# halajun/diasss

Hardware: NVIDIA B200
Metric: image-pairs/sec (extract+match) (higher is better)
Workload: dtype u8

## Files before the change

diasss_b200/csrc/fast.cu:

```cuda
#include <cuda.h>
#include <cuda_fp16.h>
#include <cuda_pipeline.h>

#include <algorithm>
#include <cstring>
#include <vector>

#include "dsx_internal.cuh"

namespace dsx {

namespace {

#ifndef DSX_FAST_WARPS
#define DSX_FAST_WARPS 8
#endif
constexpr int kWarps = DSX_FAST_WARPS;
constexpr int kLX = 8 * kWarps;
constexpr int kLXs = (kWarps == 8) ? 6 : (kWarps == 4) ? 5 : 4;
static_assert((1 << kLXs) == kLX, "kWarps must be 2, 4 or 8");
constexpr int kPad = 4;

#ifndef DSX_FAST_FP16
#define DSX_FAST_FP16 1
#endif
#ifndef DSX_FAST_END_FMA
#define DSX_FAST_END_FMA 8
#endif

__device__ __forceinline__ uint32_t ld4(const uint8_t* s, int off) {
    const uint32_t* w = reinterpret_cast<const uint32_t*>(s + (off & ~3));
    return __funnelshift_r(w[0], w[1], (off & 3) * 8);
}

template <int S>
__device__ __forceinline__ uint32_t win(uint32_t P, uint32_t Q, uint32_t N) {
    if (S == 0) return P;
    if (S < 4) return __funnelshift_r(P, Q, 8 * S);
    if (S == 4) return Q;
    if (S < 8) return __funnelshift_r(Q, N, 8 * (S - 4));
    return N;
}

#if !DSX_FAST_FP16
__device__ __forceinline__ uint32_t arc_pair(const uint32_t (&r)[16], uint32_t c, uint32_t t_floor) {
    uint32_t pn[8], px[8];
#pragma unroll
    for (int j = 0; j < 8; j++) {
        pn[j] = __vminu2(r[2 * j + 1], r[(2 * j + 2) & 15]);
        px[j] = __vmaxu2(r[2 * j + 1], r[(2 * j + 2) & 15]);
    }
    uint32_t qn[8], qx[8];
#pragma unroll
    for (int j = 0; j < 8; j++) {
        qn[j] = __vminu2(pn[j], pn[(j + 1) & 7]);
        qx[j] = __vmaxu2(px[j], px[(j + 1) & 7]);
    }
    uint32_t wn[8], wx[8];
#pragma unroll
    for (int j = 0; j < 8; j++) {
        const uint32_t en = __vmaxu2(r[2 * j], r[(2 * j + 9) & 15]), ex = __vminu2(r[2 * j], r[(2 * j + 9) & 15]);
        wn[j] = __vimin3_u16x2(qn[j], qn[(j + 2) & 7], en);
        wx[j] = __vimax3_u16x2(qx[j], qx[(j + 2) & 7], ex);
    }
    uint32_t a = __vimax3_u16x2(__vimax3_u16x2(wn[0], wn[1], wn[2]), __vimax3_u16x2(wn[3], wn[4], wn[5]), __vmaxu2(wn[6], wn[7]));
    uint32_t b = __vimin3_u16x2(__vimin3_u16x2(wx[0], wx[1], wx[2]), __vimin3_u16x2(wx[3], wx[4], wx[5]), __vminu2(wx[6], wx[7]));
    const uint32_t A = __byte_perm(a, 0, 0x4341), B = __byte_perm(b, 0, 0x4341), C = __byte_perm(c, 0, 0x4341);
    const uint32_t X = A + 0x80008000u - C, Y = C + 0x80008000u - B;
    return __vimax3_u16x2(X, Y, 0x80008000u + t_floor * 0x00010001u) - 0x80018001u;
}

#endif

__device__ __forceinline__ void hminmax(uint32_t a, uint32_t b, uint32_t& mn, uint32_t& mx) {
    const __half2 ha = *reinterpret_cast<const __half2*>(&a), hb = *reinterpret_cast<const __half2*>(&b);
    const __half2 d = __hfma2_relu(hb, __float2half2_rn(-1.0f), ha);
    const __half2 hx = __hadd2(hb, d), hn = __hsub2(ha, d);
    mx = *reinterpret_cast<const uint32_t*>(&hx);
    mn = *reinterpret_cast<const uint32_t*>(&hn);
}

__device__ __forceinline__ uint32_t arc_pair_h(const uint32_t (&r)[16], uint32_t c, uint32_t floor_bits) {
    uint32_t pn[8], px[8];
#pragma unroll
    for (int j = 0; j < 8; j++) hminmax(r[2 * j + 1], r[(2 * j + 2) & 15], pn[j], px[j]);
    uint32_t qn[8], qx[8];
#pragma unroll
    for (int j = 0; j < 8; j++) {
        qn[j] = __vminu2(pn[j], pn[(j + 1) & 7]);
        qx[j] = __vmaxu2(px[j], px[(j + 1) & 7]);
    }
    uint32_t wn[8], wx[8];
#pragma unroll
    for (int j = 0; j < 8; j++) {
        uint32_t en, ex;
        if (j < DSX_FAST_END_FMA) hminmax(r[2 * j], r[(2 * j + 9) & 15], ex, en);
        else { en = __vmaxu2(r[2 * j], r[(2 * j + 9) & 15]); ex = __vminu2(r[2 * j], r[(2 * j + 9) & 15]); }
        wn[j] = __vimin3_u16x2(qn[j], qn[(j + 2) & 7], en);
        wx[j] = __vimax3_u16x2(qx[j], qx[(j + 2) & 7], ex);
    }
    const uint32_t a = __vimax3_u16x2(__vimax3_u16x2(wn[0], wn[1], wn[2]), __vimax3_u16x2(wn[3], wn[4], wn[5]), __vmaxu2(wn[6], wn[7]));
    const uint32_t b = __vimin3_u16x2(__vimin3_u16x2(wx[0], wx[1], wx[2]), __vimin3_u16x2(wx[3], wx[4], wx[5]), __vminu2(wx[6], wx[7]));
    const __half2 ha = *reinterpret_cast<const __half2*>(&a), hb = *reinterpret_cast<const __half2*>(&b);
    const __half2 hc = *reinterpret_cast<const __half2*>(&c);
    const __half2 k256 = __float2half2_rn(256.0f);
    const __half2 X = __hadd2(ha, __hsub2(k256, hc)), Y = __hsub2(__hadd2(hc, k256), hb);
    const uint32_t m = __vimax3_u16x2(*reinterpret_cast<const uint32_t*>(&X), *reinterpret_cast<const uint32_t*>(&Y), floor_bits);
    const __half2 sc = __hadd2(*reinterpret_cast<const __half2*>(&m), __float2half2_rn(767.0f));
    return *reinterpret_cast<const uint32_t*>(&sc);
}

__device__ __forceinline__ void zero_score_border(uint8_t* score, int SP, int hd, int tid) {
    const int W = SP >> 2;
    uint32_t* sc = reinterpret_cast<uint32_t*>(score);
    for (int i = tid; i < 2 * W; i += kWarps * 32) sc[i < W ? i : (hd + 1) * W + (i - W)] = 0;
}

#ifdef DSX_FAST_PROFILE
__device__ unsigned long long g_fast_prof[512][16];
#define FAST_MARK(ph) do { if ((threadIdx.x & 31) == 0) { const long long t_ = clock64(); unsigned long long* s_ = g_fast_prof[(blockIdx.x * 8 + (threadIdx.x >> 5) + blockIdx.y * 37) & 511]; atomicAdd(s_ + 2 * (ph), (unsigned long long)(t_ - t_prev)); atomicAdd(s_ + 2 * (ph) + 1, 1ull); t_prev = t_; } } while (0)
#else
#define FAST_MARK(ph) do { } while (0)
#endif

struct FastArgs {
    LevelGeom g;
    const uint8_t* img;
    long long img_stride;
    int pitch;
    int32_t* cell_count;
    uint32_t* stage;
    long long cells_total, stage_total;
    int ini_th, min_th;
    int SP;
    int strip_bytes, score_bytes, list_bytes;
    int32_t* hist;
    unsigned long long* gbest;
    long long hist_total;
    const uint16_t* xlut;
    const uint8_t* ylut;
    int use_tma;
    CUtensorMap tmap;
};

constexpr int kFastMaxLevels = 8;
struct FastArgsAll {
    FastArgs lv[kFastMaxLevels];
    int first[kFastMaxLevels + 1];
    int nlevels;
};

__device__ __forceinline__ uint32_t smem_u32(const void* p) { return (uint32_t)__cvta_generic_to_shared(p); }

template <int SPC>
__global__ void __launch_bounds__(kWarps * 32, 32 / kWarps) fast_cells_kernel(const __grid_constant__ FastArgsAll AA) {
    int level = 0;
    while (level + 1 < AA.nlevels && (int)blockIdx.x >= AA.first[level + 1]) level++;
    const FastArgs& A = AA.lv[level];
    const int bx = (int)blockIdx.x - AA.first[level];
    extern __shared__ __align__(128) uint8_t smem[];
    __shared__ __align__(8) unsigned long long tma_bar;
#ifdef DSX_FAST_PROFILE
    long long t_prev = clock64();
#endif
    const LevelGeom& g = A.g;
    const int groupsX = (g.nCols + kWarps - 1) / kWarps;
    const int ci = bx / groupsX;
    const int j0 = (bx % groupsX) * kWarps;
    const int iniY = kMinBorder + ci * g.hCell;
    if (iniY >= g.maxBY - 3) return;
    const int maxY = min(iniY + g.hCell + 6, g.maxBY);
    const int hROI = maxY - iniY, hd = hROI - 6;
    int ncell = min(kWarps, g.nCols - j0);
    while (ncell > 0 && kMinBorder + (j0 + ncell - 1) * g.wCell >= g.maxBX - 6) ncell--;
    if (ncell == 0 || hd <= 0) return;
    const int xBegin = kMinBorder + j0 * g.wCell;
    const int xEnd = min(kMinBorder + (j0 + ncell) * g.wCell + 6, g.maxBX);
    const int xa = xBegin & ~3;
    const int xorg = A.use_tma ? ((xa - kPad) & ~15) : (xa - kPad);
    const int SP = SPC ? SPC : A.SP;
    uint8_t* strip = smem;
#if DSX_FAST_FP16
    uint8_t* score = smem;
    uint32_t* planeE = reinterpret_cast<uint32_t*>(smem + A.strip_bytes);
    uint32_t* planeO = planeE + (A.strip_bytes >> 1);
#else
    uint8_t* score = smem + 4 * A.strip_bytes;
#endif
    const uint8_t* img = A.img + (long long)blockIdx.y * A.img_stride;
    const int tid = threadIdx.x;

    if (A.use_tma == 2) {
        const uint32_t bar = smem_u32(&tma_bar);
        if (tid == 0) {
            asm volatile("mbarrier.init.shared::cta.b64 [%0], 1;" ::"r"(bar));
            asm volatile("fence.mbarrier_init.release.cluster;" ::: "memory");
            asm volatile("mbarrier.arrive.expect_tx.shared::cta.b64 _, [%0], %1;" ::"r"(bar), "r"((uint32_t)(SP * (g.hCell + 6))) : "memory");
            asm volatile("cp.async.bulk.tensor.3d.shared::cluster.global.mbarrier::complete_tx::bytes [%0], [%1, {%2, %3, %4}], [%5];"
                         ::"r"(smem_u32(strip)), "l"(&A.tmap), "r"(xorg >> 2), "r"(iniY), "r"((int)blockIdx.y), "r"(bar) : "memory");
        }
#if !DSX_FAST_FP16
        zero_score_border(score, SP, hd, tid);
#endif
        __syncthreads();
        if (tid < 32) {
            uint32_t done = 0;
            while (!done)
                asm volatile("{\n .reg .pred p;\n mbarrier.try_wait.parity.shared::cta.b64 p, [%1], %2;\n selp.u32 %0, 1, 0, p;\n}"
                             : "=r"(done) : "r"(bar), "r"(0u) : "memory");
        }
    } else if (A.use_tma) {
        const uint32_t bar = smem_u32(&tma_bar);
        const uint32_t row_bytes = (uint32_t)min(SP, A.pitch - xorg);
        if (tid == 0) {
            asm volatile("mbarrier.init.shared::cta.b64 [%0], 1;" ::"r"(bar));
            asm volatile("fence.mbarrier_init.release.cluster;" ::: "memory");
            asm volatile("mbarrier.arrive.expect_tx.shared::cta.b64 _, [%0], %1;" ::"r"(bar), "r"(row_bytes * (uint32_t)hROI) : "memory");
        }
        __syncthreads();
        if (tid < 32)
            for (int r = tid; r < hROI; r += 32)
                asm volatile("cp.async.bulk.shared::cluster.global.mbarrier::complete_tx::bytes [%0], [%1], %2, [%3];"
                             ::"r"(smem_u32(strip + r * SP)), "l"(img + (long long)(iniY + r) * A.pitch + xorg), "r"(row_bytes), "r"(bar) : "memory");
#if !DSX_FAST_FP16
        zero_score_border(score, SP, hd, tid);
#endif
        if (tid < 32) {
            uint32_t done = 0;
            while (!done)
                asm volatile("{\n .reg .pred p;\n mbarrier.try_wait.parity.shared::cta.b64 p, [%1], %2;\n selp.u32 %0, 1, 0, p;\n}"
                             : "=r"(done) : "r"(bar), "r"(0u) : "memory");
        }
    } else {
        const int nwords = (xEnd - xa + 3) >> 2;
        const int total = nwords * hROI;
        const int step_r = (kWarps * 32) / nwords, step_w = (kWarps * 32) - step_r * nwords;
        int r = tid / nwords, w = tid - r * nwords;
        for (int e = tid; e < total; e += kWarps * 32) {
            __pipeline_memcpy_async(strip + r * SP + (xa - xorg) + 4 * w, img + (long long)(iniY + r) * A.pitch + xa + 4 * w, 4);
            r += step_r; w += step_w;
            if (w >= nwords) { w -= nwords; r++; }
        }
        __pipeline_commit();
#if !DSX_FAST_FP16
        zero_score_border(score, SP, hd, tid);
#endif
        __pipeline_wait_prior(0);
    }
    FAST_MARK(0);
    __syncthreads();
    FAST_MARK(1);

#if DSX_FAST_FP16
    {
        const uint32_t* s0 = reinterpret_cast<const uint32_t*>(strip);
        const int total = (SP >> 2) * hROI;
        const uint32_t K = 0x64646464u;
        for (int e = tid; e < total; e += kWarps * 32) {
            const uint32_t a = s0[e], b = s0[e + 1];
            uint2 E, O;
            E.x = __byte_perm(a, K, 0x4140); E.y = __byte_perm(a, K, 0x4342);
            O.x = __byte_perm(a, K, 0x4241); O.y = __byte_perm(__byte_perm(a, b, 0x0043), K, 0x4140);
            *reinterpret_cast<uint2*>(planeE + 2 * e) = E;
            *reinterpret_cast<uint2*>(planeO + 2 * e) = O;
        }
    }
    FAST_MARK(2);
    __syncthreads();
    FAST_MARK(3);
    zero_score_border(score, SP, hd, tid);

    const uint32_t t_lo = (uint32_t)max(min(A.ini_th, A.min_th), 1);
    {
        constexpr int kPX = kWarps * 16;
        const int d0 = xBegin + 3 - xorg, d1 = xEnd - 3 - xorg;
        const int p0 = d0 >> 1, npx = ((d1 + 1) >> 1) - p0;
        const int W2 = SP >> 1;
        const __half2 fl = __float2half2_rn((float)(t_lo + 256));
        const uint32_t floor_bits = *reinterpret_cast<const uint32_t*>(&fl);
        for (int px = tid & (kPX - 1); px < npx; px += kPX) {
            const int e = p0 + px;
            uint32_t keep = 0xffffu;
            if (2 * e < d0) keep &= 0xff00u;
            if (2 * e + 1 >= d1) keep &= 0x00ffu;
            const int half = (hd + 1) >> 1;
            const int rbeg = (tid / kPX) ? half : 0, rend = (tid / kPX) ? hd : half;
            const uint32_t* qe = planeE + (rbeg + 3) * W2 + e;
            const uint32_t* qo = planeO + (rbeg + 3) * W2 + e;
            uint16_t* o = reinterpret_cast<uint16_t*>(score + (rbeg + 1) * SP) + e;
            uint32_t Rm = qo[-W2 + 1], Rc = qo[1], Lm = qo[-W2 - 2], Lc = qo[-2];
#pragma unroll 3
            for (int row = rbeg; row < rend; row++, qe += W2, qo += W2, o += SP >> 1) {
                uint32_t r[16];
                const uint32_t Rp = qo[W2 + 1], Lp = qo[W2 - 2];
#define RING(k, dx, dy) r[k] = ((dx) & 1) ? qo[(dy) * W2 + (((dx) - 1) >> 1)] : qe[(dy) * W2 + ((dx) >> 1)];
                RING(0, 0, 3)   RING(1, 1, 3)   RING(2, 2, 2)    r[3] = Rp;
                r[4] = Rc;      r[5] = Rm;      RING(6, 2, -2)   RING(7, 1, -3)
                RING(8, 0, -3)  RING(9, -1, -3) RING(10, -2, -2) r[11] = Lm;
                r[12] = Lc;     r[13] = Lp;     RING(14, -2, 2)  RING(15, -1, 3)
#undef RING
                const uint32_t sc = arc_pair_h(r, qe[0], floor_bits);
                *o = (uint16_t)(__byte_perm(sc, 0, 0x4420) & keep);
                Rm = Rc; Rc = Rp; Lm = Lc; Lc = Lp;
            }
        }
    }
#else
    {
        const uint32_t* s0 = reinterpret_cast<const uint32_t*>(strip);
        const int cw = A.strip_bytes >> 2;
        uint32_t* s1 = reinterpret_cast<uint32_t*>(strip) + cw;
        const int total = (SP >> 2) * hROI;
        for (int e = tid; e < total; e += kWarps * 32) {
            const uint32_t a = s0[e], b = s0[e + 1];
            s1[e] = __funnelshift_r(a, b, 8);
            s1[e + cw] = __funnelshift_r(a, b, 16);
            s1[e + 2 * cw] = __funnelshift_r(a, b, 24);
        }
    }
    FAST_MARK(2);
    __syncthreads();
    FAST_MARK(3);

    const uint32_t t_lo = (uint32_t)max(min(A.ini_th, A.min_th), 1);
    {
        const int d0 = xBegin + 3 - xorg, d1 = xEnd - 3 - xorg;
        const int w0 = d0 >> 2, nwx = ((d1 + 3) >> 2) - w0;
        const int W = SP >> 2, CW = A.strip_bytes >> 2;
        for (int wx = tid & (kLX - 1); wx < nwx; wx += kLX) {
            const int col = (w0 + wx) << 2;
            uint32_t keep = 0xffffffffu;
            if (d0 - col > 0) keep &= 0xffffffffu << (8 * (d0 - col));
            if (d1 - col < 4) keep &= 0xffffffffu >> (8 * (4 - (d1 - col)));
            const uint32_t* q = reinterpret_cast<const uint32_t*>(strip + ((tid >> kLXs) + 3) * SP + col);
            uint32_t* o = reinterpret_cast<uint32_t*>(score + ((tid >> kLXs) + 1) * SP + col);
            for (int row = tid >> kLXs; row < hd; row += (kWarps * 32) >> kLXs, q += 4 * W, o += 4 * W) {
                uint32_t ro[16], re[16];
#define WIN(S, dy) q[((S) & 3) * CW + (dy) * W + ((S) >> 2) - 1]
#define RING(k, dx, dy) { ro[k] = WIN(4 + (dx), dy); re[k] = WIN(3 + (dx), dy); }
                RING(0, 0, 3)   RING(1, 1, 3)   RING(2, 2, 2)    RING(3, 3, 1)
                RING(4, 3, 0)   RING(5, 3, -1)  RING(6, 2, -2)   RING(7, 1, -3)
                RING(8, 0, -3)  RING(9, -1, -3) RING(10, -2, -2) RING(11, -3, -1)
                RING(12, -3, 0) RING(13, -3, 1) RING(14, -2, 2)  RING(15, -1, 3)
#undef RING
                const uint32_t co = WIN(4, 0), ce = WIN(3, 0);
#undef WIN
                const uint32_t se = arc_pair(re, ce, t_lo);
                const uint32_t so = arc_pair(ro, co, t_lo);
                *o = (so * 256u + se) & keep;
            }
        }
    }
#endif
    FAST_MARK(4);
    __syncthreads();
    FAST_MARK(5);

    const int warp = tid >> 5, lane = tid & 31;
    if (warp >= ncell) return;
    const int cj = j0 + warp;
    const int iniX = kMinBorder + cj * g.wCell;
    const int maxX = min(iniX + g.wCell + 6, g.maxBX);
    const int wd = (maxX - iniX) - 6;
    const long long cell = g.cell_base + (long long)ci * g.nCols + cj;
    int32_t* out_count = A.cell_count + (long long)blockIdx.y * A.cells_total + cell;
    uint32_t* out_stage = A.stage + (long long)blockIdx.y * A.stage_total + g.stage_base +
                          ((long long)ci * g.nCols + cj) * g.cell_cap;
    if (wd <= 0) return;
    uint16_t* clist = reinterpret_cast<uint16_t*>(smem + A.strip_bytes + warp * A.list_bytes);
    const int sc0 = SP + (iniX + 3 - xorg);

    int ncorner = 0;
    const int nw = (wd + 3) >> 2;
    const uint32_t tail_mask = (wd & 3) ? ((1u << (8 * (wd & 3))) - 1u) : 0xffffffffu;
    for (int rbase = 0; rbase < hd; rbase += 32) {
        const int row = rbase + lane;
        uint32_t m_lo = 0, m_hi = 0;
        if (row < hd) {
            const int rb = sc0 + row * SP;
            uint32_t prev = 0, v = ld4(score, rb);
            if (nw == 1) v &= tail_mask;
            for (int wx = 0; wx < nw; wx++) {
                uint32_t next = 0;
                if (wx + 1 < nw) { next = ld4(score, rb + 4 * wx + 4); if (wx + 2 == nw) next &= tail_mask; }
                const uint32_t yl = __funnelshift_r(prev, v, 24), yr = __funnelshift_r(v, next, 8);
                const uint32_t xl = v & 0x7f7f7f7fu;
                const uint32_t tl = (yl | 0x80808080u) - xl, tr = (yr | 0x80808080u) - xl;
                const uint32_t gel = (yl & ~v) | (~(yl ^ v) & tl), ger = (yr & ~v) | (~(yr ^ v) & tr);
                const uint32_t gt = ~(gel | ger) & 0x80808080u;
                const uint32_t nib = (((gt >> 7) * 0x00204081u) >> 21) & 0xfu;
                if (wx < 8) m_lo |= nib << (4 * wx); else m_hi |= nib << (4 * wx - 32);
                prev = v; v = next;
            }
        }
        const int cnt = __popc(m_lo) + __popc(m_hi);
        int incl = cnt;
#pragma unroll
        for (int o = 1; o < 32; o <<= 1) { const int t = __shfl_up_sync(0xffffffffu, incl, o); if (lane >= o) incl += t; }
        int pos = ncorner + incl - cnt;
        while (m_lo) { clist[pos++] = (uint16_t)((row << 6) | (__ffs(m_lo) - 1)); m_lo &= m_lo - 1; }
        while (m_hi) { clist[pos++] = (uint16_t)((row << 6) | (__ffs(m_hi) + 31)); m_hi &= m_hi - 1; }
        ncorner += __shfl_sync(0xffffffffu, incl, 31);
    }
    __syncwarp();

    int cnt = 0;
    for (int pass = 0; pass < 2 && cnt == 0; pass++) {
        const int th = pass ? A.min_th : A.ini_th;
        for (int base = 0; base < ncorner; base += 32) {
            const int i = base + lane;
            bool emit = false; int idx = 0, s = 0;
            if (i < ncorner) {
                idx = clist[i];
                const int lx = idx & 63;
                const uint8_t* q = score + sc0 + (idx >> 6) * SP + lx;
                s = q[0];
                if (s >= th) {
                    const bool hasl = lx > 0, hasr = lx < wd - 1;
                    const int l0 = hasl ? q[-SP - 1] : 0, l2 = hasl ? q[SP - 1] : 0;
                    const int r0 = hasr ? q[-SP + 1] : 0, r2 = hasr ? q[SP + 1] : 0;
                    emit = s > l0 && s > l2 && s > r0 && s > r2 && s > q[-SP] && s > q[SP];
                }
            }
            const unsigned b = __ballot_sync(0xffffffffu, emit);
            if (emit) {
                const int e = cnt + __popc(b & ((1u << lane) - 1));
                out_stage[e] = (uint32_t)((idx & 63) + 3) | ((uint32_t)((idx >> 6) + 3) << 8) | ((uint32_t)s << 16);
                clist[e] = (uint16_t)idx;
            }
            cnt += __popc(b);
        }
        __syncwarp();
    }
    {
        int32_t* hist = A.hist + (long long)blockIdx.y * A.hist_total + g.hist_base;
        unsigned long long* gbest = A.gbest + (long long)blockIdx.y * A.hist_total + g.hist_base;
        const int ox = cj * g.wCell + 3, oy = ci * g.hCell + 3;
        const unsigned long long cl = (unsigned long long)(ci * g.nCols + cj);
        for (int base = 0; base < cnt; base += 32) {
            const int e = base + lane;
            unsigned code = 0xffffffffu, v = 0;
            if (e < cnt) {
                const int idx = clist[e];
                const unsigned xl = __ldg(A.xlut + ox + (idx & 63));
                code = ((xl >> 8) << (2 * g.qt_depth)) + ((unsigned)__ldg(A.ylut + oy + (idx >> 6)) << g.qt_depth) + (xl & 0xff);
                v = ((unsigned)score[sc0 + (idx >> 6) * SP + (idx & 63)] << 12) | (unsigned)(0xfff - e);
            }
            const unsigned peers = __match_any_sync(0xffffffffu, code);
            const unsigned mv = __reduce_max_sync(peers, v);
            if (e < cnt && lane == __ffs(peers) - 1) {
                atomicAdd(hist + code, __popc(peers));
                atomicMax(gbest + code, ((unsigned long long)(mv >> 12) << 56) | (kBestOrderMask - ((cl << 12) | (0xfff - (mv & 0xfff)))));
            }
        }
    }
    if (lane == 0) *out_count = cnt;
    FAST_MARK(6);
}

}

int fast_profile_read(unsigned long long* out16, int reset) {
#ifdef DSX_FAST_PROFILE
    std::vector<unsigned long long> h(512 * 16);
    if (cudaMemcpyFromSymbol(h.data(), g_fast_prof, sizeof(unsigned long long) * h.size()) != cudaSuccess) return DSX_ERR_CUDA;
    for (int k = 0; k < 16; k++) { out16[k] = 0; for (int s = 0; s < 512; s++) out16[k] += h[s * 16 + k]; }
    if (reset) {
        std::fill(h.begin(), h.end(), 0ull);
        if (cudaMemcpyToSymbol(g_fast_prof, h.data(), sizeof(unsigned long long) * h.size()) != cudaSuccess) return DSX_ERR_CUDA;
    }
    return DSX_OK;
#else
    (void)out16; (void)reset;
    set_error("built without DSX_FAST_PROFILE");
    return DSX_ERR_INVALID;
#endif
}

namespace {
typedef CUresult (*EncodeTiledFn)(CUtensorMap*, CUtensorMapDataType, cuuint32_t, void*, const cuuint64_t*, const cuuint64_t*,
                                  const cuuint32_t*, const cuuint32_t*, CUtensorMapInterleave, CUtensorMapSwizzle,
                                  CUtensorMapL2promotion, CUtensorMapFloatOOBfill);
EncodeTiledFn encode_tiled() {
    static EncodeTiledFn fn = [] {
        void* p = nullptr;
        cudaDriverEntryPointQueryResult q;
        if (cudaGetDriverEntryPoint("cuTensorMapEncodeTiled", &p, cudaEnableDefault, &q) != cudaSuccess || q != cudaDriverEntryPointSuccess) p = nullptr;
        cudaGetLastError();
        return (EncodeTiledFn)p;
    }();
    return fn;
}
}

bool make_plane_map(CUtensorMap* m, const uint8_t* base, int pitch, int rows, long long img_stride, int n, int SP, int box_rows) {
    EncodeTiledFn enc = encode_tiled();
    if (!enc || SP / 4 > 256 || box_rows > 256) return false;
    const cuuint64_t dims[3] = {(cuuint64_t)(pitch / 4), (cuuint64_t)rows, (cuuint64_t)n};
    const cuuint64_t strides[2] = {(cuuint64_t)pitch, (cuuint64_t)img_stride};
    const cuuint32_t box[3] = {(cuuint32_t)(SP / 4), (cuuint32_t)box_rows, 1};
    const cuuint32_t estr[3] = {1, 1, 1};
    return enc(m, CU_TENSOR_MAP_DATA_TYPE_UINT32, 3, (void*)base, dims, strides, box, estr, CU_TENSOR_MAP_INTERLEAVE_NONE,
               CU_TENSOR_MAP_SWIZZLE_NONE, CU_TENSOR_MAP_L2_PROMOTION_NONE, CU_TENSOR_MAP_FLOAT_OOB_FILL_NONE) == CUDA_SUCCESS;
}

int launch_fast(dsx_ctx* ctx, const uint8_t* images, size_t step, size_t img_stride, int n) {
    StageTimer _t(ctx, 1);
    const ShapePlan& P = ctx->plan;
    DSX_CUDA(cudaMemsetAsync(ctx->ws.cell_count, 0, sizeof(int32_t) * (size_t)n * P.cells_total, ctx->stream));
    DSX_CUDA(cudaMemsetAsync(ctx->ws.hist, 0, sizeof(int32_t) * (size_t)n * P.hist_total, ctx->stream));
    DSX_CUDA(cudaMemsetAsync(ctx->ws.gbest, 0, sizeof(unsigned long long) * (size_t)n * P.hist_total, ctx->stream));
    auto level_sp = [&](int l) { return ((((kWarps * P.lv[l].wCell + 6 + 3 + 3) & ~3) + kPad + 8 + 12) + 15) & ~15; };
    int sp_launch = 0;
    auto fill = [&](int l, FastArgs& A) -> size_t {
        const LevelGeom& g = P.lv[l];
        A.g = g;
        A.img = (l == 0) ? images : ctx->ws.pyr + g.offset;
        A.img_stride = (l == 0) ? (long long)img_stride : P.pyr_bytes;
        A.pitch = (l == 0) ? (int)step : g.pitch;
        A.cell_count = ctx->ws.cell_count; A.stage = ctx->ws.stage;
        A.cells_total = P.cells_total; A.stage_total = P.stage_total;
        A.hist = ctx->ws.hist; A.gbest = ctx->ws.gbest; A.hist_total = P.hist_total;
        A.xlut = P.d_xlut + g.lut_x; A.ylut = P.d_ylut + g.lut_y;
        A.ini_th = std::min(std::max(ctx->p.ini_th_fast, 0), 255);
        A.min_th = std::min(std::max(ctx->p.min_th_fast, 0), 255);
        A.SP = sp_launch;
        A.strip_bytes = ((A.SP * (g.hCell + 6) + 16) + 15) & ~15;
        A.score_bytes = ((A.SP * (g.hCell + 2) + 16) + 15) & ~15;
        A.list_bytes = ((((g.wCell + 1) / 2) * g.hCell * 2) + 15) & ~15;
        A.use_tma = (ctx->fast_tma && ((uintptr_t)A.img & 15) == 0 && (A.pitch & 15) == 0 && (A.img_stride & 15) == 0) ? 1 : 0;
        memset(&A.tmap, 0, sizeof(A.tmap));
        if (A.use_tma && ctx->fast_tma >= 2 && make_plane_map(&A.tmap, A.img, A.pitch, g.rows, A.img_stride, n, A.SP, g.hCell + 6))
            A.use_tma = 2;
#if DSX_FAST_FP16
        return (size_t)5 * A.strip_bytes;
#else
        return (size_t)4 * A.strip_bytes + A.score_bytes;
#endif
    };
    for (int l0 = 0; l0 < P.nlevels; l0 += kFastMaxLevels) {
        FastArgsAll AA;
        memset(&AA, 0, sizeof(AA));
        size_t smem = 0;
        int nl = 0, blocks = 0;
        sp_launch = 0;
        for (int l = l0; l < std::min(P.nlevels, l0 + kFastMaxLevels); l++)
            if (P.lv[l].n_cells) sp_launch = std::max(sp_launch, level_sp(l));
        for (int l = l0; l < std::min(P.nlevels, l0 + kFastMaxLevels); l++) {
            const LevelGeom& g = P.lv[l];
            if (g.n_cells == 0) continue;
            FastArgs& A = AA.lv[nl];
            const size_t sm = fill(l, A);
            if ((size_t)kWarps * A.list_bytes > (size_t)(DSX_FAST_FP16 ? 4 : 3) * A.strip_bytes) { set_error("FAST corner lists do not fit the strip copies"); return DSX_ERR_INVALID; }
            if (sm > 200 * 1024) { set_error("FAST cell too large for shared memory"); return DSX_ERR_INVALID; }
            smem = std::max(smem, sm);
            AA.first[nl] = blocks;
            blocks += g.nRows * ((g.nCols + kWarps - 1) / kWarps);
            nl++;
        }
        if (nl == 0) continue;
        AA.first[nl] = blocks;
        AA.nlevels = nl;
        dim3 grid(blocks, n);
        auto launch = [&](auto kernel) -> int {
            if (smem > 48 * 1024) DSX_CUDA(cudaFuncSetAttribute(kernel, cudaFuncAttributeMaxDynamicSharedMemorySize, (int)smem));
            kernel<<<grid, kWarps * 32, smem, ctx->stream>>>(AA);
            return DSX_OK;
        };
        int rc;
        switch (sp_launch) {
            case 288: rc = launch(fast_cells_kernel<288>); break;
            case 304: rc = launch(fast_cells_kernel<304>); break;
            default:  rc = launch(fast_cells_kernel<0>); break;
        }
        if (rc != DSX_OK) return rc;
        DSX_LAUNCH_CHECK();
    }
    return DSX_OK;
}

}
```

Baseline: 152,600.

## Add FAST four-point pretest with warp-compacted exact scoring and fallback rescoring

When the initial FAST threshold is at least 4, each pixel pair is first screened with the cardinal four-point test at ini_th. Only pixels that pass go into a per-warp shared-memory queue, and the full 16-point arc score is computed for them in dense 32-wide batches. All other pixels get a floor score written directly. If a cell finds no corners at ini_th, its scores are recomputed from global memory at the lower threshold before the min_th sweep. This aims to skip most full ring evaluations, at the cost of queue bookkeeping, extra shared memory and a possibly expensive rescore path for sparse cells.

```diff
diff --git a/diasss_b200/csrc/fast.cu b/diasss_b200/csrc/fast.cu
--- a/diasss_b200/csrc/fast.cu
+++ b/diasss_b200/csrc/fast.cu
@@ -27,6 +27,10 @@
 #ifndef DSX_FAST_END_FMA
 #define DSX_FAST_END_FMA 8
 #endif
+
+constexpr int kPretestMinTh = 4;
+constexpr int kChunk = 6;
+constexpr int kQueueCap = (31 + 32 * kChunk + 7) & ~7;
 
 __device__ __forceinline__ uint32_t ld4(const uint8_t* s, int off) {
     const uint32_t* w = reinterpret_cast<const uint32_t*>(s + (off & ~3));
@@ -108,6 +112,28 @@
     const uint32_t m = __vimax3_u16x2(*reinterpret_cast<const uint32_t*>(&X), *reinterpret_cast<const uint32_t*>(&Y), floor_bits);
     const __half2 sc = __hadd2(*reinterpret_cast<const __half2*>(&m), __float2half2_rn(767.0f));
     return *reinterpret_cast<const uint32_t*>(&sc);
+}
+
+__device__ void rescore_cell(uint8_t* sc, int SP, const uint8_t* p, int pitch, int wd, int hd, uint32_t t_floor, int lane) {
+    const __half2 fl = __float2half2_rn((float)(t_floor + 256));
+    const uint32_t floor_bits = *reinterpret_cast<const uint32_t*>(&fl);
+    const int npr = (wd + 1) >> 1;
+    for (int k = lane; k < npr * hd; k += 32) {
+        const int ly = k / npr, lx = 2 * (k - ly * npr);
+        const int d2 = (lx + 1 < wd) ? 1 : 0;
+        const uint8_t* q = p + (long long)ly * pitch + lx;
+        uint32_t r[16];
+#define PX2(dx, dy) (0x64006400u | q[(dy) * pitch + (dx)] | ((uint32_t)q[(dy) * pitch + (dx) + d2] << 16))
+        r[0] = PX2(0, 3);    r[1] = PX2(1, 3);    r[2] = PX2(2, 2);    r[3] = PX2(3, 1);
+        r[4] = PX2(3, 0);    r[5] = PX2(3, -1);   r[6] = PX2(2, -2);   r[7] = PX2(1, -3);
+        r[8] = PX2(0, -3);   r[9] = PX2(-1, -3);  r[10] = PX2(-2, -2); r[11] = PX2(-3, -1);
+        r[12] = PX2(-3, 0);  r[13] = PX2(-3, 1);  r[14] = PX2(-2, 2);  r[15] = PX2(-1, 3);
+        const uint32_t s = arc_pair_h(r, PX2(0, 0), floor_bits);
+#undef PX2
+        uint8_t* o = sc + ly * SP + lx;
+        o[0] = (uint8_t)s;
+        if (d2) o[1] = (uint8_t)(s >> 16);
+    }
 }
 
 __device__ __forceinline__ void zero_score_border(uint8_t* score, int SP, int hd, int tid) {
@@ -271,37 +297,111 @@
     zero_score_border(score, SP, hd, tid);
 
     const uint32_t t_lo = (uint32_t)max(min(A.ini_th, A.min_th), 1);
+    const bool pretest = A.ini_th >= kPretestMinTh;
     {
         constexpr int kPX = kWarps * 16;
         const int d0 = xBegin + 3 - xorg, d1 = xEnd - 3 - xorg;
         const int p0 = d0 >> 1, npx = ((d1 + 1) >> 1) - p0;
         const int W2 = SP >> 1;
-        const __half2 fl = __float2half2_rn((float)(t_lo + 256));
-        const uint32_t floor_bits = *reinterpret_cast<const uint32_t*>(&fl);
-        for (int px = tid & (kPX - 1); px < npx; px += kPX) {
-            const int e = p0 + px;
-            uint32_t keep = 0xffffu;
-            if (2 * e < d0) keep &= 0xff00u;
-            if (2 * e + 1 >= d1) keep &= 0x00ffu;
-            const int half = (hd + 1) >> 1;
-            const int rbeg = (tid / kPX) ? half : 0, rend = (tid / kPX) ? hd : half;
-            const uint32_t* qe = planeE + (rbeg + 3) * W2 + e;
-            const uint32_t* qo = planeO + (rbeg + 3) * W2 + e;
-            uint16_t* o = reinterpret_cast<uint16_t*>(score + (rbeg + 1) * SP) + e;
-            uint32_t Rm = qo[-W2 + 1], Rc = qo[1], Lm = qo[-W2 - 2], Lc = qo[-2];
+        const int half = (hd + 1) >> 1;
+        const int rbeg = (tid / kPX) ? half : 0, rend = (tid / kPX) ? hd : half;
+        if (pretest) {
+            const __half2 fl = __float2half2_rn((float)(A.ini_th + 256)), hT = __float2half2_rn((float)A.ini_th);
+            const uint32_t floor_bits = *reinterpret_cast<const uint32_t*>(&fl);
+            const uint32_t floor_pair = (uint32_t)(A.ini_th - 1) * 0x0101u;
+            const int lane = tid & 31;
+            uint16_t* queue = reinterpret_cast<uint16_t*>(smem + 5 * A.strip_bytes) + (tid >> 5) * kQueueCap;
+            for (int pxb = (tid & (kPX - 1)) & ~31; pxb < npx; pxb += kPX) {
+                const int eb = p0 + pxb;
+                const bool live = pxb + lane < npx;
+                uint32_t keep = 0xffffu;
+                if (2 * (eb + lane) < d0) keep &= 0xff00u;
+                if (2 * (eb + lane) + 1 >= d1) keep &= 0x00ffu;
+                const uint32_t* qe = planeE + (rbeg + 3) * W2 + eb + lane;
+                const uint32_t* qo = planeO + (rbeg + 3) * W2 + eb + lane;
+                uint16_t* o = reinterpret_cast<uint16_t*>(score + (rbeg + 1) * SP) + eb + lane;
+                const uint16_t fw = (uint16_t)(floor_pair & keep);
+                auto exact = [&](int ent) {
+                    const int row = ent >> 5, e = eb + (ent & 31);
+                    const uint32_t* pe = planeE + (row + 3) * W2 + e;
+                    const uint32_t* po = planeO + (row + 3) * W2 + e;
+                    uint32_t r[16];
+#define RING(k, dx, dy) r[k] = ((dx) & 1) ? po[(dy) * W2 + (((dx) - 1) >> 1)] : pe[(dy) * W2 + ((dx) >> 1)];
+                    RING(0, 0, 3)   RING(1, 1, 3)   RING(2, 2, 2)    RING(3, 3, 1)
+                    RING(4, 3, 0)   RING(5, 3, -1)  RING(6, 2, -2)   RING(7, 1, -3)
+                    RING(8, 0, -3)  RING(9, -1, -3) RING(10, -2, -2) RING(11, -3, -1)
+                    RING(12, -3, 0) RING(13, -3, 1) RING(14, -2, 2)  RING(15, -1, 3)
+#undef RING
+                    uint32_t k = 0xffffu;
+                    if (2 * e < d0) k &= 0xff00u;
+                    if (2 * e + 1 >= d1) k &= 0x00ffu;
+                    const uint32_t sc = arc_pair_h(r, pe[0], floor_bits);
+                    reinterpret_cast<uint16_t*>(score + (row + 1) * SP)[e] = (uint16_t)(__byte_perm(sc, 0, 0x4420) & k);
+                };
+                int nq = 0;
+                for (int r0 = rbeg; r0 < rend; r0 += kChunk) {
+                    const int r1 = min(r0 + kChunk, rend);
+                    uint32_t bits = 0;
+                    if (live) {
+                        for (int row = r0; row < r1; row++, qe += W2, qo += W2, o += SP >> 1) {
+                            const uint32_t c = qe[0], r0w = qe[3 * W2], r4 = qo[1], r8 = qe[-3 * W2], r12 = qo[-2];
+                            uint32_t n04, x04, n812, x812;
+                            hminmax(r0w, r4, n04, x04);
+                            hminmax(r8, r12, n812, x812);
+                            const uint32_t a = __vimax3_u16x2(n04, n812, __vmaxu2(__vminu2(r4, r8), __vminu2(r12, r0w)));
+                            const uint32_t b = __vimin3_u16x2(x04, x812, __vminu2(__vmaxu2(r4, r8), __vmaxu2(r12, r0w)));
+                            const __half2 hc = *reinterpret_cast<const __half2*>(&c);
+                            const __half2 ha = *reinterpret_cast<const __half2*>(&a), hb = *reinterpret_cast<const __half2*>(&b);
+                            const bool pass = !__hble2(ha, __hadd2(hc, hT)) | !__hbge2(hb, __hsub2(hc, hT));
+                            bits |= (uint32_t)pass << (row - r0);
+                            *o = fw;
+                        }
+                    }
+                    const int cnt = __popc(bits);
+                    int incl = cnt;
+#pragma unroll
+                    for (int d = 1; d < 32; d <<= 1) { const int t = __shfl_up_sync(0xffffffffu, incl, d); if (lane >= d) incl += t; }
+                    const int total = nq + __shfl_sync(0xffffffffu, incl, 31);
+                    for (int pos = nq + incl - cnt; bits; bits &= bits - 1)
+                        queue[pos++] = (uint16_t)(((r0 + __ffs(bits) - 1) << 5) | lane);
+                    __syncwarp();
+                    int done = 0;
+                    for (; done + 32 <= total; done += 32) exact(queue[done + lane]);
+                    nq = total - done;
+                    const int ent = (lane < nq) ? queue[done + lane] : 0;
+                    __syncwarp();
+                    if (lane < nq) queue[lane] = (uint16_t)ent;
+                    __syncwarp();
+                }
+                if (lane < nq) exact(queue[lane]);
+                __syncwarp();
+            }
+        } else {
+            const __half2 fl = __float2half2_rn((float)(t_lo + 256));
+            const uint32_t floor_bits = *reinterpret_cast<const uint32_t*>(&fl);
+            for (int px = tid & (kPX - 1); px < npx; px += kPX) {
+                const int e = p0 + px;
+                uint32_t keep = 0xffffu;
+                if (2 * e < d0) keep &= 0xff00u;
+                if (2 * e + 1 >= d1) keep &= 0x00ffu;
+                const uint32_t* qe = planeE + (rbeg + 3) * W2 + e;
+                const uint32_t* qo = planeO + (rbeg + 3) * W2 + e;
+                uint16_t* o = reinterpret_cast<uint16_t*>(score + (rbeg + 1) * SP) + e;
+                uint32_t Rm = qo[-W2 + 1], Rc = qo[1], Lm = qo[-W2 - 2], Lc = qo[-2];
 #pragma unroll 3
-            for (int row = rbeg; row < rend; row++, qe += W2, qo += W2, o += SP >> 1) {
-                uint32_t r[16];
-                const uint32_t Rp = qo[W2 + 1], Lp = qo[W2 - 2];
+                for (int row = rbeg; row < rend; row++, qe += W2, qo += W2, o += SP >> 1) {
+                    uint32_t r[16];
+                    const uint32_t Rp = qo[W2 + 1], Lp = qo[W2 - 2];
 #define RING(k, dx, dy) r[k] = ((dx) & 1) ? qo[(dy) * W2 + (((dx) - 1) >> 1)] : qe[(dy) * W2 + ((dx) >> 1)];
-                RING(0, 0, 3)   RING(1, 1, 3)   RING(2, 2, 2)    r[3] = Rp;
-                r[4] = Rc;      r[5] = Rm;      RING(6, 2, -2)   RING(7, 1, -3)
-                RING(8, 0, -3)  RING(9, -1, -3) RING(10, -2, -2) r[11] = Lm;
-                r[12] = Lc;     r[13] = Lp;     RING(14, -2, 2)  RING(15, -1, 3)
+                    RING(0, 0, 3)   RING(1, 1, 3)   RING(2, 2, 2)    r[3] = Rp;
+                    r[4] = Rc;      r[5] = Rm;      RING(6, 2, -2)   RING(7, 1, -3)
+                    RING(8, 0, -3)  RING(9, -1, -3) RING(10, -2, -2) r[11] = Lm;
+                    r[12] = Lc;     r[13] = Lp;     RING(14, -2, 2)  RING(15, -1, 3)
 #undef RING
-                const uint32_t sc = arc_pair_h(r, qe[0], floor_bits);
-                *o = (uint16_t)(__byte_perm(sc, 0, 0x4420) & keep);
-                Rm = Rc; Rc = Rp; Lm = Lc; Lc = Lp;
+                    const uint32_t sc = arc_pair_h(r, qe[0], floor_bits);
+                    *o = (uint16_t)(__byte_perm(sc, 0, 0x4420) & keep);
+                    Rm = Rc; Rc = Rp; Lm = Lc; Lc = Lp;
+                }
             }
         }
     }
@@ -323,6 +423,7 @@
     FAST_MARK(3);
 
     const uint32_t t_lo = (uint32_t)max(min(A.ini_th, A.min_th), 1);
+    constexpr bool pretest = false;
     {
         const int d0 = xBegin + 3 - xorg, d1 = xEnd - 3 - xorg;
         const int w0 = d0 >> 2, nwx = ((d1 + 3) >> 2) - w0;
@@ -370,43 +471,45 @@
     uint16_t* clist = reinterpret_cast<uint16_t*>(smem + A.strip_bytes + warp * A.list_bytes);
     const int sc0 = SP + (iniX + 3 - xorg);
 
-    int ncorner = 0;
     const int nw = (wd + 3) >> 2;
     const uint32_t tail_mask = (wd & 3) ? ((1u << (8 * (wd & 3))) - 1u) : 0xffffffffu;
-    for (int rbase = 0; rbase < hd; rbase += 32) {
-        const int row = rbase + lane;
-        uint32_t m_lo = 0, m_hi = 0;
-        if (row < hd) {
-            const int rb = sc0 + row * SP;
-            uint32_t prev = 0, v = ld4(score, rb);
-            if (nw == 1) v &= tail_mask;
-            for (int wx = 0; wx < nw; wx++) {
-                uint32_t next = 0;
-                if (wx + 1 < nw) { next = ld4(score, rb + 4 * wx + 4); if (wx + 2 == nw) next &= tail_mask; }
-                const uint32_t yl = __funnelshift_r(prev, v, 24), yr = __funnelshift_r(v, next, 8);
-                const uint32_t xl = v & 0x7f7f7f7fu;
-                const uint32_t tl = (yl | 0x80808080u) - xl, tr = (yr | 0x80808080u) - xl;
-                const uint32_t gel = (yl & ~v) | (~(yl ^ v) & tl), ger = (yr & ~v) | (~(yr ^ v) & tr);
-                const uint32_t gt = ~(gel | ger) & 0x80808080u;
-                const uint32_t nib = (((gt >> 7) * 0x00204081u) >> 21) & 0xfu;
-                if (wx < 8) m_lo |= nib << (4 * wx); else m_hi |= nib << (4 * wx - 32);
-                prev = v; v = next;
-            }
-        }
-        const int cnt = __popc(m_lo) + __popc(m_hi);
-        int incl = cnt;
-#pragma unroll
-        for (int o = 1; o < 32; o <<= 1) { const int t = __shfl_up_sync(0xffffffffu, incl, o); if (lane >= o) incl += t; }
-        int pos = ncorner + incl - cnt;
-        while (m_lo) { clist[pos++] = (uint16_t)((row << 6) | (__ffs(m_lo) - 1)); m_lo &= m_lo - 1; }
-        while (m_hi) { clist[pos++] = (uint16_t)((row << 6) | (__ffs(m_hi) + 31)); m_hi &= m_hi - 1; }
-        ncorner += __shfl_sync(0xffffffffu, incl, 31);
-    }
-    __syncwarp();
-
-    int cnt = 0;
-    for (int pass = 0; pass < 2 && cnt == 0; pass++) {
-        const int th = pass ? A.min_th : A.ini_th;
+    auto list_corners = [&]() -> int {
+        int ncorner = 0;
+        for (int rbase = 0; rbase < hd; rbase += 32) {
+            const int row = rbase + lane;
+            uint32_t m_lo = 0, m_hi = 0;
+            if (row < hd) {
+                const int rb = sc0 + row * SP;
+                uint32_t prev = 0, v = ld4(score, rb);
+                if (nw == 1) v &= tail_mask;
+                for (int wx = 0; wx < nw; wx++) {
+                    uint32_t next = 0;
+                    if (wx + 1 < nw) { next = ld4(score, rb + 4 * wx + 4); if (wx + 2 == nw) next &= tail_mask; }
+                    const uint32_t yl = __funnelshift_r(prev, v, 24), yr = __funnelshift_r(v, next, 8);
+                    const uint32_t xl = v & 0x7f7f7f7fu;
+                    const uint32_t tl = (yl | 0x80808080u) - xl, tr = (yr | 0x80808080u) - xl;
+                    const uint32_t gel = (yl & ~v) | (~(yl ^ v) & tl), ger = (yr & ~v) | (~(yr ^ v) & tr);
+                    const uint32_t gt = ~(gel | ger) & 0x80808080u;
+                    const uint32_t nib = (((gt >> 7) * 0x00204081u) >> 21) & 0xfu;
+                    if (wx < 8) m_lo |= nib << (4 * wx); else m_hi |= nib << (4 * wx - 32);
+                    prev = v; v = next;
+                }
+            }
+            const int cnt = __popc(m_lo) + __popc(m_hi);
+            int incl = cnt;
+#pragma unroll
+            for (int o = 1; o < 32; o <<= 1) { const int t = __shfl_up_sync(0xffffffffu, incl, o); if (lane >= o) incl += t; }
+            int pos = ncorner + incl - cnt;
+            while (m_lo) { clist[pos++] = (uint16_t)((row << 6) | (__ffs(m_lo) - 1)); m_lo &= m_lo - 1; }
+            while (m_hi) { clist[pos++] = (uint16_t)((row << 6) | (__ffs(m_hi) + 31)); m_hi &= m_hi - 1; }
+            ncorner += __shfl_sync(0xffffffffu, incl, 31);
+        }
+        __syncwarp();
+        return ncorner;
+    };
+
+    auto sweep = [&](int ncorner, int th) -> int {
+        int cnt = 0;
         for (int base = 0; base < ncorner; base += 32) {
             const int i = base + lane;
             bool emit = false; int idx = 0, s = 0;
@@ -431,6 +534,20 @@
             cnt += __popc(b);
         }
         __syncwarp();
+        return cnt;
+    };
+
+    int ncorner = list_corners();
+    int cnt = sweep(ncorner, A.ini_th);
+    if (cnt == 0) {
+#if DSX_FAST_FP16
+        if (pretest) {
+            rescore_cell(score + sc0, SP, img + (long long)(iniY + 3) * A.pitch + iniX + 3, A.pitch, wd, hd, t_lo, lane);
+            __syncwarp();
+            ncorner = list_corners();
+        }
+#endif
+        cnt = sweep(ncorner, A.min_th);
     }
     {
         int32_t* hist = A.hist + (long long)blockIdx.y * A.hist_total + g.hist_base;
@@ -533,7 +650,7 @@
         if (A.use_tma && ctx->fast_tma >= 2 && make_plane_map(&A.tmap, A.img, A.pitch, g.rows, A.img_stride, n, A.SP, g.hCell + 6))
             A.use_tma = 2;
 #if DSX_FAST_FP16
-        return (size_t)5 * A.strip_bytes;
+        return (size_t)5 * A.strip_bytes + (size_t)kWarps * kQueueCap * 2;
 #else
         return (size_t)4 * A.strip_bytes + A.score_bytes;
 #endif
```

Result: slower. 146,200, median of 6 (-4.2%).

## Add compass pre-test to skip full FAST arc scoring for most pixels

Applied to the files above, without the earlier changes.

Before computing the full 16-pixel arc score, each pixel is screened with a cheap 4-point compass bound against the initial threshold. Only pixels that pass are queued per warp in shared memory and rescored with a single-direction exact arc kernel. If the fallback lower threshold pass is needed, the cell is rescored exactly from global memory, and the corner-list build moves inside the per-pass loop. This targets the dense per-pixel ring evaluation, at the cost of warp queueing, shuffles and divergence, plus extra work whenever a cell falls back to the lower threshold.

```diff
diff --git a/diasss_b200/csrc/fast.cu b/diasss_b200/csrc/fast.cu
--- a/diasss_b200/csrc/fast.cu
+++ b/diasss_b200/csrc/fast.cu
@@ -109,6 +109,60 @@
     const __half2 sc = __hadd2(*reinterpret_cast<const __half2*>(&m), __float2half2_rn(767.0f));
     return *reinterpret_cast<const uint32_t*>(&sc);
 }
+
+#if DSX_FAST_FP16
+__device__ __forceinline__ void compass_bound_h(uint32_t n, uint32_t e, uint32_t s, uint32_t w, uint32_t c, uint32_t th_bits,
+                                                bool& up, bool& dn) {
+    uint32_t nsn, nsx, ewn, ewx;
+    hminmax(n, s, nsn, nsx);
+    hminmax(e, w, ewn, ewx);
+    const uint32_t a = __vminu2(nsx, ewx), b = __vmaxu2(nsn, ewn);
+    const __half2 ha = *reinterpret_cast<const __half2*>(&a), hb = *reinterpret_cast<const __half2*>(&b);
+    const __half2 hc = *reinterpret_cast<const __half2*>(&c);
+    const __half2 k256 = __float2half2_rn(256.0f);
+    const __half2 X = __hadd2(ha, __hsub2(k256, hc)), Y = __hsub2(__hadd2(hc, k256), hb);
+    up = __vmaxu2(*reinterpret_cast<const uint32_t*>(&X), th_bits) != th_bits;
+    dn = __vmaxu2(*reinterpret_cast<const uint32_t*>(&Y), th_bits) != th_bits;
+}
+
+__device__ __forceinline__ uint32_t hmin2(uint32_t a, uint32_t b) { uint32_t mn, mx; hminmax(a, b, mn, mx); return mn; }
+__device__ __forceinline__ uint32_t hmax2(uint32_t a, uint32_t b) { uint32_t mn, mx; hminmax(a, b, mn, mx); return mx; }
+
+template <bool UP>
+__device__ __forceinline__ uint32_t arc_pair_h1(const uint32_t (&r)[16], uint32_t c, uint32_t floor_bits) {
+    uint32_t p[8], q[8], w[8];
+#pragma unroll
+    for (int j = 0; j < 8; j++) p[j] = UP ? hmin2(r[2 * j + 1], r[(2 * j + 2) & 15]) : hmax2(r[2 * j + 1], r[(2 * j + 2) & 15]);
+#pragma unroll
+    for (int j = 0; j < 8; j++) q[j] = UP ? __vminu2(p[j], p[(j + 1) & 7]) : __vmaxu2(p[j], p[(j + 1) & 7]);
+#pragma unroll
+    for (int j = 0; j < 8; j++) {
+        const uint32_t en = UP ? __vmaxu2(r[2 * j], r[(2 * j + 9) & 15]) : __vminu2(r[2 * j], r[(2 * j + 9) & 15]);
+        w[j] = UP ? __vimin3_u16x2(q[j], q[(j + 2) & 7], en) : __vimax3_u16x2(q[j], q[(j + 2) & 7], en);
+    }
+    const uint32_t a = UP ? __vimax3_u16x2(__vimax3_u16x2(w[0], w[1], w[2]), __vimax3_u16x2(w[3], w[4], w[5]), __vmaxu2(w[6], w[7]))
+                          : __vimin3_u16x2(__vimin3_u16x2(w[0], w[1], w[2]), __vimin3_u16x2(w[3], w[4], w[5]), __vminu2(w[6], w[7]));
+    const __half2 ha = *reinterpret_cast<const __half2*>(&a), hc = *reinterpret_cast<const __half2*>(&c);
+    const __half2 k256 = __float2half2_rn(256.0f);
+    const __half2 X = UP ? __hadd2(ha, __hsub2(k256, hc)) : __hsub2(__hadd2(hc, k256), ha);
+    const uint32_t m = __vmaxu2(*reinterpret_cast<const uint32_t*>(&X), floor_bits);
+    const __half2 sc = __hadd2(*reinterpret_cast<const __half2*>(&m), __float2half2_rn(767.0f));
+    return *reinterpret_cast<const uint32_t*>(&sc);
+}
+
+__host__ __device__ constexpr uint32_t h2_256_plus(uint32_t v) { return (0x5c00u + 4u * v) * 0x00010001u; }
+
+__device__ __forceinline__ uint32_t exact_score_gmem(const uint8_t* p, int pitch, uint32_t floor_bits) {
+    uint32_t r[16];
+#define RING(k, dx, dy) r[k] = 0x64006400u | ((uint32_t)__ldg(p + (dy) * pitch + (dx)) * 0x00010001u);
+    RING(0, 0, 3)   RING(1, 1, 3)   RING(2, 2, 2)    RING(3, 3, 1)
+    RING(4, 3, 0)   RING(5, 3, -1)  RING(6, 2, -2)   RING(7, 1, -3)
+    RING(8, 0, -3)  RING(9, -1, -3) RING(10, -2, -2) RING(11, -3, -1)
+    RING(12, -3, 0) RING(13, -3, 1) RING(14, -2, 2)  RING(15, -1, 3)
+#undef RING
+    return arc_pair_h(r, 0x64006400u | ((uint32_t)__ldg(p) * 0x00010001u), floor_bits) & 0xffu;
+}
+#endif
 
 __device__ __forceinline__ void zero_score_border(uint8_t* score, int SP, int hd, int tid) {
     const int W = SP >> 2;
@@ -151,6 +205,12 @@
 };
 
 __device__ __forceinline__ uint32_t smem_u32(const void* p) { return (uint32_t)__cvta_generic_to_shared(p); }
+__device__ __forceinline__ int lds_u16(uint32_t a) {
+    unsigned short v;
+    asm volatile("ld.shared.u16 %0, [%1];" : "=h"(v) : "r"(a));
+    return v;
+}
+__device__ __forceinline__ void sts_u16(uint32_t a, int v) { asm volatile("st.shared.u16 [%0], %1;" ::"r"(a), "h"((unsigned short)v)); }
 
 template <int SPC>
 __global__ void __launch_bounds__(kWarps * 32, 32 / kWarps) fast_cells_kernel(const __grid_constant__ FastArgsAll AA) {
@@ -160,6 +220,9 @@
     const int bx = (int)blockIdx.x - AA.first[level];
     extern __shared__ __align__(128) uint8_t smem[];
     __shared__ __align__(8) unsigned long long tma_bar;
+#if DSX_FAST_FP16
+    __shared__ uint16_t fast_queue[kWarps][2][64];
+#endif
 #ifdef DSX_FAST_PROFILE
     long long t_prev = clock64();
 #endif
@@ -271,38 +334,83 @@
     zero_score_border(score, SP, hd, tid);
 
     const uint32_t t_lo = (uint32_t)max(min(A.ini_th, A.min_th), 1);
+    const uint32_t floor_bits = h2_256_plus(t_lo);
     {
         constexpr int kPX = kWarps * 16;
         const int d0 = xBegin + 3 - xorg, d1 = xEnd - 3 - xorg;
         const int p0 = d0 >> 1, npx = ((d1 + 1) >> 1) - p0;
         const int W2 = SP >> 1;
-        const __half2 fl = __float2half2_rn((float)(t_lo + 256));
-        const uint32_t floor_bits = *reinterpret_cast<const uint32_t*>(&fl);
-        for (int px = tid & (kPX - 1); px < npx; px += kPX) {
-            const int e = p0 + px;
-            uint32_t keep = 0xffffu;
-            if (2 * e < d0) keep &= 0xff00u;
-            if (2 * e + 1 >= d1) keep &= 0x00ffu;
-            const int half = (hd + 1) >> 1;
-            const int rbeg = (tid / kPX) ? half : 0, rend = (tid / kPX) ? hd : half;
+        const int OE = (int)(planeO - planeE);
+        const uint32_t th_bits = h2_256_plus((uint32_t)A.ini_th);
+        const uint32_t floor_word = (t_lo - 1) * 0x0101u;
+        const int lane = tid & 31;
+        const unsigned lanes_below = (1u << lane) - 1u;
+        const uint32_t qa = smem_u32(fast_queue[tid >> 5][0]);
+        const int half = (hd + 1) >> 1;
+        const int rbeg = (tid / kPX) ? half : 0, rend = (tid / kPX) ? hd : half;
+        auto exact = [&](bool up, int v, int e0, uint32_t keep) {
+            const int row = v >> 5, e = e0 + (v & 31);
+            const uint32_t* qe = planeE + (row + 3) * W2 + e;
+            const uint32_t* qo = qe + OE;
+            uint32_t r[16];
+#define RING(k, dx, dy) r[k] = ((dx) & 1) ? qo[(dy) * W2 + (((dx) - 1) >> 1)] : qe[(dy) * W2 + ((dx) >> 1)];
+            RING(0, 0, 3)   RING(1, 1, 3)   RING(2, 2, 2)    RING(3, 3, 1)
+            RING(4, 3, 0)   RING(5, 3, -1)  RING(6, 2, -2)   RING(7, 1, -3)
+            RING(8, 0, -3)  RING(9, -1, -3) RING(10, -2, -2) RING(11, -3, -1)
+            RING(12, -3, 0) RING(13, -3, 1) RING(14, -2, 2)  RING(15, -1, 3)
+#undef RING
+            const uint32_t sc = up ? arc_pair_h1<true>(r, qe[0], floor_bits) : arc_pair_h1<false>(r, qe[0], floor_bits);
+            uint16_t* o = reinterpret_cast<uint16_t*>(score + (row + 1) * SP + 2 * e);
+            const uint32_t old = __byte_perm((uint32_t)*o, 0, 0x4140);
+            *o = (uint16_t)(__byte_perm(__vmaxu2(old, sc & 0x00ff00ffu), 0, 0x4420) & keep);
+        };
+        auto flush = [&](bool up, int& n, int e0, uint32_t keep) {
+            n -= 32;
+            __syncwarp();
+            const int v = lds_u16(qa + (up ? 0 : 128) + 2 * (n + lane));
+            __syncwarp();
+            exact(up, v, e0, __shfl_sync(0xffffffffu, keep, v & 31));
+        };
+        for (int pb = (tid & (kPX - 1)) & ~31; pb < npx; pb += kPX) {
+            const int e0 = p0 + pb;
+            const int e = min(e0 + lane, p0 + npx - 1);
+            uint32_t keep = 0;
+            if (pb + lane < npx) {
+                keep = 0xffffu;
+                if (2 * e < d0) keep &= 0xff00u;
+                if (2 * e + 1 >= d1) keep &= 0x00ffu;
+            }
+            const uint32_t floor_keep = floor_word & keep;
             const uint32_t* qe = planeE + (rbeg + 3) * W2 + e;
-            const uint32_t* qo = planeO + (rbeg + 3) * W2 + e;
+            const uint32_t* qo = qe + OE;
             uint16_t* o = reinterpret_cast<uint16_t*>(score + (rbeg + 1) * SP) + e;
-            uint32_t Rm = qo[-W2 + 1], Rc = qo[1], Lm = qo[-W2 - 2], Lc = qo[-2];
-#pragma unroll 3
-            for (int row = rbeg; row < rend; row++, qe += W2, qo += W2, o += SP >> 1) {
-                uint32_t r[16];
+            uint32_t Rc = qo[1], Lc = qo[-2];
+            int nu = 0, nd = 0;
+            int tag = (rbeg << 5) | lane;
+#pragma unroll 2
+            for (int row = rbeg; row < rend; row++, qe += W2, qo += W2, o += SP >> 1, tag += 32) {
                 const uint32_t Rp = qo[W2 + 1], Lp = qo[W2 - 2];
-#define RING(k, dx, dy) r[k] = ((dx) & 1) ? qo[(dy) * W2 + (((dx) - 1) >> 1)] : qe[(dy) * W2 + ((dx) >> 1)];
-                RING(0, 0, 3)   RING(1, 1, 3)   RING(2, 2, 2)    r[3] = Rp;
-                r[4] = Rc;      r[5] = Rm;      RING(6, 2, -2)   RING(7, 1, -3)
-                RING(8, 0, -3)  RING(9, -1, -3) RING(10, -2, -2) r[11] = Lm;
-                r[12] = Lc;     r[13] = Lp;     RING(14, -2, 2)  RING(15, -1, 3)
-#undef RING
-                const uint32_t sc = arc_pair_h(r, qe[0], floor_bits);
-                *o = (uint16_t)(__byte_perm(sc, 0, 0x4420) & keep);
-                Rm = Rc; Rc = Rp; Lm = Lc; Lc = Lp;
-            }
+                bool up, dn;
+                compass_bound_h(qe[3 * W2], Rc, qe[-3 * W2], Lc, qe[0], th_bits, up, dn);
+                up &= keep != 0; dn &= keep != 0;
+                if (keep) *o = (uint16_t)floor_keep;
+                const unsigned bu = __ballot_sync(0xffffffffu, up), bd = __ballot_sync(0xffffffffu, dn);
+                if (up) sts_u16(qa + 2 * (nu + __popc(bu & lanes_below)), tag);
+                if (dn) sts_u16(qa + 128 + 2 * (nd + __popc(bd & lanes_below)), tag);
+                nu += __popc(bu); nd += __popc(bd);
+                if (nu >= 32) flush(true, nu, e0, keep);
+                if (nd >= 32) flush(false, nd, e0, keep);
+                Rc = Rp; Lc = Lp;
+            }
+            __syncwarp();
+            int v = lds_u16(qa + 2 * lane);
+            uint32_t kv = __shfl_sync(0xffffffffu, keep, v & 31);
+            if (lane < nu) exact(true, v, e0, kv);
+            __syncwarp();
+            v = lds_u16(qa + 128 + 2 * lane);
+            kv = __shfl_sync(0xffffffffu, keep, v & 31);
+            if (lane < nd) exact(false, v, e0, kv);
+            __syncwarp();
         }
     }
 #else
@@ -370,43 +478,53 @@
     uint16_t* clist = reinterpret_cast<uint16_t*>(smem + A.strip_bytes + warp * A.list_bytes);
     const int sc0 = SP + (iniX + 3 - xorg);
 
-    int ncorner = 0;
     const int nw = (wd + 3) >> 2;
     const uint32_t tail_mask = (wd & 3) ? ((1u << (8 * (wd & 3))) - 1u) : 0xffffffffu;
-    for (int rbase = 0; rbase < hd; rbase += 32) {
-        const int row = rbase + lane;
-        uint32_t m_lo = 0, m_hi = 0;
-        if (row < hd) {
-            const int rb = sc0 + row * SP;
-            uint32_t prev = 0, v = ld4(score, rb);
-            if (nw == 1) v &= tail_mask;
-            for (int wx = 0; wx < nw; wx++) {
-                uint32_t next = 0;
-                if (wx + 1 < nw) { next = ld4(score, rb + 4 * wx + 4); if (wx + 2 == nw) next &= tail_mask; }
-                const uint32_t yl = __funnelshift_r(prev, v, 24), yr = __funnelshift_r(v, next, 8);
-                const uint32_t xl = v & 0x7f7f7f7fu;
-                const uint32_t tl = (yl | 0x80808080u) - xl, tr = (yr | 0x80808080u) - xl;
-                const uint32_t gel = (yl & ~v) | (~(yl ^ v) & tl), ger = (yr & ~v) | (~(yr ^ v) & tr);
-                const uint32_t gt = ~(gel | ger) & 0x80808080u;
-                const uint32_t nib = (((gt >> 7) * 0x00204081u) >> 21) & 0xfu;
-                if (wx < 8) m_lo |= nib << (4 * wx); else m_hi |= nib << (4 * wx - 32);
-                prev = v; v = next;
-            }
-        }
-        const int cnt = __popc(m_lo) + __popc(m_hi);
-        int incl = cnt;
-#pragma unroll
-        for (int o = 1; o < 32; o <<= 1) { const int t = __shfl_up_sync(0xffffffffu, incl, o); if (lane >= o) incl += t; }
-        int pos = ncorner + incl - cnt;
-        while (m_lo) { clist[pos++] = (uint16_t)((row << 6) | (__ffs(m_lo) - 1)); m_lo &= m_lo - 1; }
-        while (m_hi) { clist[pos++] = (uint16_t)((row << 6) | (__ffs(m_hi) + 31)); m_hi &= m_hi - 1; }
-        ncorner += __shfl_sync(0xffffffffu, incl, 31);
-    }
-    __syncwarp();
-
     int cnt = 0;
     for (int pass = 0; pass < 2 && cnt == 0; pass++) {
         const int th = pass ? A.min_th : A.ini_th;
+#if DSX_FAST_FP16
+        if (pass) {
+            const uint8_t* p0 = img + (long long)(iniY + 3) * A.pitch + (iniX + 3);
+            for (int i = lane; i < hd * wd; i += 32) {
+                const int ly = i / wd, lx = i - ly * wd;
+                score[sc0 + ly * SP + lx] = (uint8_t)exact_score_gmem(p0 + (long long)ly * A.pitch + lx, A.pitch, floor_bits);
+            }
+            __syncwarp();
+        }
+#endif
+        int ncorner = 0;
+        for (int rbase = 0; rbase < hd; rbase += 32) {
+            const int row = rbase + lane;
+            uint32_t m_lo = 0, m_hi = 0;
+            if (row < hd) {
+                const int rb = sc0 + row * SP;
+                uint32_t prev = 0, v = ld4(score, rb);
+                if (nw == 1) v &= tail_mask;
+                for (int wx = 0; wx < nw; wx++) {
+                    uint32_t next = 0;
+                    if (wx + 1 < nw) { next = ld4(score, rb + 4 * wx + 4); if (wx + 2 == nw) next &= tail_mask; }
+                    const uint32_t yl = __funnelshift_r(prev, v, 24), yr = __funnelshift_r(v, next, 8);
+                    const uint32_t xl = v & 0x7f7f7f7fu;
+                    const uint32_t tl = (yl | 0x80808080u) - xl, tr = (yr | 0x80808080u) - xl;
+                    const uint32_t gel = (yl & ~v) | (~(yl ^ v) & tl), ger = (yr & ~v) | (~(yr ^ v) & tr);
+                    const uint32_t gt = ~(gel | ger) & 0x80808080u;
+                    const uint32_t nib = (((gt >> 7) * 0x00204081u) >> 21) & 0xfu;
+                    if (wx < 8) m_lo |= nib << (4 * wx); else m_hi |= nib << (4 * wx - 32);
+                    prev = v; v = next;
+                }
+            }
+            const int nrow = __popc(m_lo) + __popc(m_hi);
+            int incl = nrow;
+#pragma unroll
+            for (int o = 1; o < 32; o <<= 1) { const int t = __shfl_up_sync(0xffffffffu, incl, o); if (lane >= o) incl += t; }
+            int pos = ncorner + incl - nrow;
+            while (m_lo) { clist[pos++] = (uint16_t)((row << 6) | (__ffs(m_lo) - 1)); m_lo &= m_lo - 1; }
+            while (m_hi) { clist[pos++] = (uint16_t)((row << 6) | (__ffs(m_hi) + 31)); m_hi &= m_hi - 1; }
+            ncorner += __shfl_sync(0xffffffffu, incl, 31);
+        }
+        __syncwarp();
+
         for (int base = 0; base < ncorner; base += 32) {
             const int i = base + lane;
             bool emit = false; int idx = 0, s = 0;
```

Result: no change. 152,600 before, 151,900 after (median of 6 runs) (-0.4%).
